# wesselb/stheno

Measured on NVIDIA H100. Metric: log-marginal-likelihoods/sec (n=16384 fp64 EQ), higher is better.
Workload: dtype f64

## Files before the change

stheno_b200/csrc/common.cuh:

```cuda
#pragma once
#include <cuda_runtime.h>
#include <stdint.h>

#include <atomic>
#include <mutex>

#include "../../include/gpk.h"

namespace gpk {

extern long long g_launch_count;

inline int cuda_rc(cudaError_t e) { return e == cudaSuccess ? 0 : -1000 - (int)e; }

#define GPK_CHECK_LAUNCH()                                                  \
  do {                                                                      \
    if (const int rc__ = ::gpk::cuda_rc(cudaGetLastError())) return rc__; \
  } while (0)

#define GPK_COUNT_LAUNCH() (++::gpk::g_launch_count)

template <auto Kernel>
int opt_in_smem(int bytes) {
  static std::atomic<int> set[64];
  static std::mutex mu;
  int dev = 0;
  if (const int rc = cuda_rc(cudaGetDevice(&dev))) return rc;
  if (dev >= 64) return GPK_ERR_UNSUPPORTED;
  if (bytes <= set[dev].load(std::memory_order_acquire)) return 0;
  std::lock_guard<std::mutex> lock(mu);
  if (bytes <= set[dev].load(std::memory_order_relaxed)) return 0;
  if (const int rc = cuda_rc(cudaFuncSetAttribute(Kernel, cudaFuncAttributeMaxDynamicSharedMemorySize, bytes))) return rc;
  set[dev].store(bytes, std::memory_order_release);
  return 0;
}

template <typename T>
__device__ __forceinline__ T t_exp(T v) {
  return sizeof(T) == 8 ? (T)exp((double)v) : (T)expf((float)v);
}
template <typename T>
__device__ __forceinline__ T t_sqrt(T v) {
  return sizeof(T) == 8 ? (T)sqrt((double)v) : (T)sqrtf((float)v);
}
template <typename T>
__device__ __forceinline__ T t_rsqrt(T v) {
  return sizeof(T) == 8 ? (T)rsqrt((double)v) : (T)rsqrtf((float)v);
}
template <typename T>
__device__ __forceinline__ T t_log(T v) {
  return sizeof(T) == 8 ? (T)log((double)v) : (T)logf((float)v);
}

__device__ __forceinline__ uint32_t smem_u32(const void* p) {
  return static_cast<uint32_t>(__cvta_generic_to_shared(p));
}

__device__ __forceinline__ void cp_async16(void* smem_dst, const void* gmem_src) {
  asm volatile("cp.async.cg.shared.global [%0], [%1], 16;\n" ::"r"(smem_u32(smem_dst)), "l"(gmem_src));
}
__device__ __forceinline__ void cp_async_commit() { asm volatile("cp.async.commit_group;\n" ::); }
template <int N>
__device__ __forceinline__ void cp_async_wait() {
  asm volatile("cp.async.wait_group %0;\n" ::"n"(N));
}

__device__ __forceinline__ void mbar_init(uint64_t* bar, uint32_t count) {
  asm volatile("mbarrier.init.shared::cta.b64 [%0], %1;\n" ::"r"(smem_u32(bar)), "r"(count));
}
__device__ __forceinline__ void fence_mbar_init() { asm volatile("fence.mbarrier_init.release.cluster;\n" ::); }
__device__ __forceinline__ void fence_proxy_async() { asm volatile("fence.proxy.async.shared::cta;\n" ::); }
__device__ __forceinline__ void mbar_arrive_expect_tx(uint64_t* bar, uint32_t bytes) {
  asm volatile("mbarrier.arrive.expect_tx.shared::cta.b64 _, [%0], %1;\n" ::"r"(smem_u32(bar)), "r"(bytes));
}
__device__ __forceinline__ void mbar_wait(uint64_t* bar, uint32_t phase) {
  asm volatile(
      "{\n"
      ".reg .pred P1;\n"
      "WAIT_LOOP:\n"
      "mbarrier.try_wait.parity.shared::cta.b64 P1, [%0], %1;\n"
      "@P1 bra WAIT_DONE;\n"
      "bra WAIT_LOOP;\n"
      "WAIT_DONE:\n"
      "}\n" ::"r"(smem_u32(bar)),
      "r"(phase)
      : "memory");
}
__device__ __forceinline__ uint32_t cluster_ctarank() {
  uint32_t r;
  asm volatile("mov.u32 %0, %%cluster_ctarank;\n" : "=r"(r));
  return r;
}
__device__ __forceinline__ void cluster_sync() {
  asm volatile("barrier.cluster.arrive.release;\nbarrier.cluster.wait.acquire;\n" ::: "memory");
}
__device__ __forceinline__ void mbar_arrive_cluster(uint64_t* bar, uint32_t rank) {
  asm volatile(
      "{\n"
      ".reg .b32 remote;\n"
      "mapa.shared::cluster.u32 remote, %0, %1;\n"
      "mbarrier.arrive.shared::cluster.b64 _, [remote];\n"
      "}\n" ::"r"(smem_u32(bar)),
      "r"(rank)
      : "memory");
}
__device__ __forceinline__ void tma_load_3d_multicast(void* dst, const void* map, int c0, int c1, int c2, uint64_t* bar,
                                                      uint16_t cta_mask) {
  asm volatile(
      "cp.async.bulk.tensor.3d.shared::cluster.global.mbarrier::complete_tx::bytes.multicast::cluster [%0], [%1, {%2, %3, "
      "%4}], [%5], %6;\n" ::"r"(smem_u32(dst)),
      "l"(map), "r"(c0), "r"(c1), "r"(c2), "r"(smem_u32(bar)), "h"(cta_mask)
      : "memory");
}
__device__ __forceinline__ void bulk_copy_g2s(void* smem_dst, const void* gmem_src, uint32_t bytes, uint64_t* bar) {
  asm volatile(
      "cp.async.bulk.shared::cluster.global.mbarrier::complete_tx::bytes [%0], [%1], %2, [%3];\n" ::"r"(
          smem_u32(smem_dst)),
      "l"(gmem_src), "r"(bytes), "r"(smem_u32(bar))
      : "memory");
}

__device__ __forceinline__ void dmma884(double& c0, double& c1, double a, double b) {
  asm("mma.sync.aligned.m8n8k4.row.col.f64.f64.f64.f64 {%0,%1}, {%2}, {%3}, {%0,%1};\n"
               : "+d"(c0), "+d"(c1)
               : "d"(a), "d"(b));
}

template <typename T>
__device__ __forceinline__ T warp_sum(T v) {
#pragma unroll
  for (int o = 16; o > 0; o >>= 1) v += __shfl_xor_sync(0xffffffffu, v, o);
  return v;
}


int kernel_rows(const gpk_kernel_desc* desc, const double* xg, int64_t xg_gstride, int64_t n, const double* yg,
                int64_t yg_gstride, int64_t n2, int32_t d, double* out, int64_t ldo, cudaStream_t stream);
int kernel_rows(const gpk_kernel_desc* desc, const float* xg, int64_t xg_gstride, int64_t n, const float* yg,
                int64_t yg_gstride, int64_t n2, int32_t d, float* out, int64_t ldo, cudaStream_t stream);

int row_dot_sq(const double* V, int64_t ldv, int64_t rows, int64_t n_cols, const double* b, double* dot, double* sq,
               cudaStream_t stream);
int row_dot_sq(const float* V, int64_t ldv, int64_t rows, int64_t n_cols, const float* b, float* dot, float* sq,
               cudaStream_t stream);

int gemm_nt(int64_t M, int64_t N, int64_t K, double alpha, const double* A, int64_t lda, int64_t a_bs, const double* B,
            int64_t ldb, int64_t b_bs, double beta, double* C, int64_t ldc, int64_t c_bs, int32_t lower, int32_t batch,
            int32_t S, void* ws, int64_t ws_bytes, cudaStream_t stream);
int gemm_nt(int64_t M, int64_t N, int64_t K, float alpha, const float* A, int64_t lda, int64_t a_bs, const float* B,
            int64_t ldb, int64_t b_bs, float beta, float* C, int64_t ldc, int64_t c_bs, int32_t lower, int32_t batch,
            int32_t S, void* ws, int64_t ws_bytes, cudaStream_t stream);
bool prof_enabled();
void prof_begin(cudaStream_t stream, double flops, int kind);
void prof_end(cudaStream_t stream);

int trsm_right(const double* L, int64_t ldl, int64_t n_pad, double* B, int64_t ldb, int64_t rows, int32_t S, void* ws,
               int64_t ws_bytes, cudaStream_t stream);
int trsm_right(const float* L, int64_t ldl, int64_t n_pad, float* B, int64_t ldb, int64_t rows, int32_t S, void* ws,
               int64_t ws_bytes, cudaStream_t stream);

int oz_check_emulation(int32_t S, const void* ws);
int64_t oz_ws_bytes(int64_t rows, int64_t K, int32_t S);
int oz_slice_panel(const double* P, int64_t ldp, int64_t rows, int64_t K, void* ws, int64_t cap_rows, int32_t S,
                   cudaStream_t stream);
int oz_gemm_sliced(int64_t M, int64_t N, int64_t K, double alpha, const void* wsA, int64_t capA, int64_t rowA,
                   const void* wsB, int64_t capB, int64_t rowB, double beta, double* C, int64_t ldc, int32_t lower,
                   int32_t S, cudaStream_t stream);
int gemm_nt_f64_emulated(int64_t M, int64_t N, int64_t K, double alpha, const double* A, int64_t lda, const double* B,
                         int64_t ldb, double beta, double* C, int64_t ldc, int32_t lower, int32_t S, void* ws,
                         int64_t ws_bytes, cudaStream_t stream);

int gemm_nt_f32_tc(int64_t M, int64_t N, int64_t K, float alpha, const float* A, int64_t lda, int64_t a_bs, const float* B,
                   int64_t ldb, int64_t b_bs, float beta, float* C, int64_t ldc, int64_t c_bs, int32_t lower,
                   int32_t batch, cudaStream_t stream);
int syrk_f64_tf32x3(int64_t M, int64_t N, int64_t K, const float* ws_rows, double* C, int64_t ldc, cudaStream_t stream);
int convert_panel_f32(const double* P, int64_t ldp, int64_t rows, int64_t K, float* ws, cudaStream_t stream);

}
```

stheno_b200/csrc/gemm.cu:

```cuda
#include <vector>

#include "common.cuh"

namespace gpk {

constexpr int GM_BM = 128, GM_BN = 128, GM_BK = 16, GM_THREADS = 256;

template <typename T>
struct GemmParams {
  int64_t M, N, K;
  T alpha, beta;
  const T* A;
  int64_t lda, a_bs;
  const T* B;
  int64_t ldb, b_bs;
  T* C;
  int64_t ldc, c_bs;
  int32_t lower;
  int32_t tiles_m, tiles_n;
};

__device__ __forceinline__ void tile_coords(int id, int tiles_m, int tiles_n, int& tm, int& tn) {
  const int GROUP = 8;
  const int per_group = GROUP * tiles_n;
  const int group = id / per_group;
  const int first_m = group * GROUP;
  const int gsize = min(tiles_m - first_m, GROUP);
  const int r = id - group * per_group;
  tm = first_m + r % gsize;
  tn = r / gsize;
}

constexpr int G2_THREADS = 512;

struct Gemm2Params {
  int64_t K;
  double alpha, beta;
  const double* A;
  int64_t lda, a_bs;
  const double* B;
  int64_t ldb, b_bs;
  double* C;
  int64_t ldc, c_bs;
  int32_t lower, tiles_m, tiles_n, n_groups;
  int32_t tiles_per_batch, total_tiles;
};

__host__ __device__ __forceinline__ int g2_lower_tiles(int rows, int tiles_n) {
  const int tri = rows < tiles_n ? rows : tiles_n;
  return tri * (tri + 1) / 2 + (rows - tri) * tiles_n;
}

__device__ __forceinline__ void g2_decode(const Gemm2Params& p, int idx, int& b, int& tm, int& tn) {
  b = idx / p.tiles_per_batch;
  int r = idx - b * p.tiles_per_batch;
  if (!p.lower) {
    tile_coords(r, p.tiles_m, p.tiles_n, tm, tn);
    return;
  }
  int g = 0;
  while (g + 1 < p.n_groups && g2_lower_tiles(8 * (g + 1), p.tiles_n) <= r) ++g;
  r -= g2_lower_tiles(8 * g, p.tiles_n);
  const int first = g * 8;
  const int gsize = min(p.tiles_m - first, 8);
  const int c0 = min(first, p.tiles_n);
  if (r < c0 * gsize) {
    tn = r / gsize;
    tm = first + r - tn * gsize;
    return;
  }
  r -= c0 * gsize;
  for (int c = 0; c < gsize; ++c) {
    const int cnt = gsize - c;
    if (r < cnt) {
      tn = first + c;
      tm = tn + r;
      return;
    }
    r -= cnt;
  }
  tn = 0;
  tm = first;
}

template <int BK, int STAGES>
__global__ void __launch_bounds__(G2_THREADS, 1) gemm_nt_f64_v2_kernel(const __grid_constant__ Gemm2Params p) {
  constexpr int K8 = BK / 8;
  constexpr int STAGE_ELEMS = GM_BM * BK;
  constexpr int RB = K8 * 64;
  constexpr int GPR = BK / 2;
  constexpr int ROWS_PER_PASS = G2_THREADS / GPR;
  constexpr int PASSES = GM_BM / ROWS_PER_PASS;
  const int tid = threadIdx.x, lane = tid & 31, warp = tid >> 5;
  const int wm = warp >> 2, wn = warp & 3;
  extern __shared__ __align__(16) double gm_smem[];
  double* As = gm_smem;
  double* Bs = gm_smem + STAGES * STAGE_ELEMS;

  const int KT = (int)(p.K / BK);
  const int my_tiles = (p.total_tiles - (int)blockIdx.x + (int)gridDim.x - 1) / (int)gridDim.x;
  const int total_iters = my_tiles * KT;

  const int ld_row = tid / GPR, ld_g = tid % GPR;
  const int ld_off = (ld_row >> 3) * RB + ((ld_g >> 2) * 32 + (ld_row & 7) * 4 + (ld_g & 3)) * 2;
  int ld_it = 0, ld_kt = 0, ld_tile = blockIdx.x, ld_slot = 0;
  const double *ld_a = nullptr, *ld_b = nullptr;
  auto load_next = [&]() {
    if (ld_it < total_iters) {
      if (ld_kt == 0) {
        int b, tm, tn;
        g2_decode(p, ld_tile, b, tm, tn);
        ld_a = p.A + (int64_t)b * p.a_bs + ((int64_t)tm * GM_BM + ld_row) * p.lda + ld_g * 2;
        ld_b = p.B + (int64_t)b * p.b_bs + ((int64_t)tn * GM_BN + ld_row) * p.ldb + ld_g * 2;
      }
      double* as = As + ld_slot * STAGE_ELEMS + ld_off;
      double* bs = Bs + ld_slot * STAGE_ELEMS + ld_off;
      const int64_t koff = (int64_t)ld_kt * BK;
#pragma unroll
      for (int i = 0; i < PASSES; ++i) {
        cp_async16(as + i * (ROWS_PER_PASS / 8) * RB, ld_a + (int64_t)i * ROWS_PER_PASS * p.lda + koff);
        cp_async16(bs + i * (ROWS_PER_PASS / 8) * RB, ld_b + (int64_t)i * ROWS_PER_PASS * p.ldb + koff);
      }
      ++ld_it;
      if (++ld_slot == STAGES) ld_slot = 0;
      if (++ld_kt == KT) {
        ld_kt = 0;
        ld_tile += gridDim.x;
      }
    }
    cp_async_commit();
  };

#pragma unroll
  for (int s = 0; s < STAGES - 1; ++s) load_next();

  double acc[4][4][2];
  int slot = 0;
  const int frag_a = (wm * 4) * RB + lane * 2, frag_b = (wn * 4) * RB + lane * 2;
  for (int t = 0; t < my_tiles; ++t) {
    int b, tm, tn;
    g2_decode(p, (int)blockIdx.x + t * (int)gridDim.x, b, tm, tn);
#pragma unroll
    for (int i = 0; i < 4; ++i)
#pragma unroll
      for (int j = 0; j < 4; ++j) acc[i][j][0] = acc[i][j][1] = 0.0;

    for (int kt = 0; kt < KT; ++kt) {
      cp_async_wait<STAGES - 2>();
      __syncthreads();
      const double* as = As + slot * STAGE_ELEMS + frag_a;
      const double* bs = Bs + slot * STAGE_ELEMS + frag_b;
#pragma unroll
      for (int k8 = 0; k8 < K8; ++k8) {
        double2 a[4], bb[4];
#pragma unroll
        for (int i = 0; i < 4; ++i) a[i] = *reinterpret_cast<const double2*>(as + i * RB + k8 * 64);
#pragma unroll
        for (int j = 0; j < 4; ++j) bb[j] = *reinterpret_cast<const double2*>(bs + j * RB + k8 * 64);
#pragma unroll
        for (int i = 0; i < 4; ++i)
#pragma unroll
          for (int j = 0; j < 4; ++j) dmma884(acc[i][j][0], acc[i][j][1], a[i].x, bb[j].x);
        if (k8 == 0) load_next();
#pragma unroll
        for (int i = 0; i < 4; ++i)
#pragma unroll
          for (int j = 0; j < 4; ++j) dmma884(acc[i][j][0], acc[i][j][1], a[i].y, bb[j].y);
      }
      if (++slot == STAGES) slot = 0;
    }

    double* Cg = p.C + (int64_t)b * p.c_bs + ((int64_t)tm * GM_BM + wm * 32 + (lane >> 2)) * p.ldc +
                 (int64_t)tn * GM_BN + wn * 32 + 2 * (lane & 3);
    const double alpha = p.alpha, beta = p.beta;
    if (beta != 0.0) {
      double2 old[4][4];
#pragma unroll
      for (int i = 0; i < 4; ++i)
#pragma unroll
        for (int j = 0; j < 4; ++j) old[i][j] = *reinterpret_cast<const double2*>(Cg + (int64_t)i * 8 * p.ldc + j * 8);
#pragma unroll
      for (int i = 0; i < 4; ++i)
#pragma unroll
        for (int j = 0; j < 4; ++j) {
          double2 v;
          v.x = fma(alpha, acc[i][j][0], beta * old[i][j].x);
          v.y = fma(alpha, acc[i][j][1], beta * old[i][j].y);
          *reinterpret_cast<double2*>(Cg + (int64_t)i * 8 * p.ldc + j * 8) = v;
        }
    } else {
#pragma unroll
      for (int i = 0; i < 4; ++i)
#pragma unroll
        for (int j = 0; j < 4; ++j)
          *reinterpret_cast<double2*>(Cg + (int64_t)i * 8 * p.ldc + j * 8) =
              make_double2(alpha * acc[i][j][0], alpha * acc[i][j][1]);
    }
  }
  cp_async_wait<0>();
}

constexpr int G3_BN = 64, G3_THREADS = 256;

template <int BK, int STAGES>
__global__ void __launch_bounds__(G3_THREADS, 2) gemm_nt_f64_v3_kernel(const GemmParams<double> p) {
  constexpr int K8 = BK / 8;
  constexpr int RB = K8 * 64;
  constexpr int A_ELEMS = GM_BM * BK, B_ELEMS = G3_BN * BK;
  constexpr int GPR = BK / 2;
  constexpr int ROWS_PER_PASS = G3_THREADS / GPR;
  constexpr int A_PASSES = GM_BM / ROWS_PER_PASS, B_PASSES = G3_BN / ROWS_PER_PASS;
  int tm, tn;
  tile_coords(blockIdx.x, p.tiles_m, p.tiles_n, tm, tn);
  if (p.lower && tn * G3_BN >= (tm + 1) * GM_BM) return;
  const int b = blockIdx.y;
  const int tid = threadIdx.x, lane = tid & 31, warp = tid >> 5;
  const int wm = warp >> 1, wn = warp & 1;
  extern __shared__ __align__(16) double gm_smem[];
  double* As = gm_smem;
  double* Bs = gm_smem + STAGES * A_ELEMS;

  const int ld_row = tid / GPR, ld_g = tid % GPR;
  const int ld_off = (ld_row >> 3) * RB + ((ld_g >> 2) * 32 + (ld_row & 7) * 4 + (ld_g & 3)) * 2;
  const double* ld_a = p.A + (int64_t)b * p.a_bs + ((int64_t)tm * GM_BM + ld_row) * p.lda + ld_g * 2;
  const double* ld_b = p.B + (int64_t)b * p.b_bs + ((int64_t)tn * G3_BN + ld_row) * p.ldb + ld_g * 2;
  const int KT = (int)(p.K / BK);
  int ld_kt = 0, ld_slot = 0;
  auto load_next = [&]() {
    if (ld_kt < KT) {
      double* as = As + ld_slot * A_ELEMS + ld_off;
      double* bs = Bs + ld_slot * B_ELEMS + ld_off;
      const int64_t koff = (int64_t)ld_kt * BK;
#pragma unroll
      for (int i = 0; i < A_PASSES; ++i)
        cp_async16(as + i * (ROWS_PER_PASS / 8) * RB, ld_a + (int64_t)i * ROWS_PER_PASS * p.lda + koff);
#pragma unroll
      for (int i = 0; i < B_PASSES; ++i)
        cp_async16(bs + i * (ROWS_PER_PASS / 8) * RB, ld_b + (int64_t)i * ROWS_PER_PASS * p.ldb + koff);
      ++ld_kt;
      if (++ld_slot == STAGES) ld_slot = 0;
    }
    cp_async_commit();
  };
#pragma unroll
  for (int s = 0; s < STAGES - 1; ++s) load_next();

  double acc[4][4][2];
#pragma unroll
  for (int i = 0; i < 4; ++i)
#pragma unroll
    for (int j = 0; j < 4; ++j) acc[i][j][0] = acc[i][j][1] = 0.0;

  int slot = 0;
  const int frag_a = (wm * 4) * RB + lane * 2, frag_b = (wn * 4) * RB + lane * 2;
  for (int kt = 0; kt < KT; ++kt) {
    cp_async_wait<STAGES - 2>();
    __syncthreads();
    const double* as = As + slot * A_ELEMS + frag_a;
    const double* bs = Bs + slot * B_ELEMS + frag_b;
#pragma unroll
    for (int k8 = 0; k8 < K8; ++k8) {
      double2 a[4], bb[4];
#pragma unroll
      for (int i = 0; i < 4; ++i) a[i] = *reinterpret_cast<const double2*>(as + i * RB + k8 * 64);
#pragma unroll
      for (int j = 0; j < 4; ++j) bb[j] = *reinterpret_cast<const double2*>(bs + j * RB + k8 * 64);
#pragma unroll
      for (int i = 0; i < 4; ++i)
#pragma unroll
        for (int j = 0; j < 4; ++j) dmma884(acc[i][j][0], acc[i][j][1], a[i].x, bb[j].x);
      if (k8 == 0) load_next();
#pragma unroll
      for (int i = 0; i < 4; ++i)
#pragma unroll
        for (int j = 0; j < 4; ++j) dmma884(acc[i][j][0], acc[i][j][1], a[i].y, bb[j].y);
    }
    if (++slot == STAGES) slot = 0;
  }
  cp_async_wait<0>();

  double* Cg = p.C + (int64_t)b * p.c_bs + ((int64_t)tm * GM_BM + wm * 32 + (lane >> 2)) * p.ldc +
               (int64_t)tn * G3_BN + wn * 32 + 2 * (lane & 3);
  const double alpha = p.alpha, beta = p.beta;
  if (beta != 0.0) {
    double2 old[4][4];
#pragma unroll
    for (int i = 0; i < 4; ++i)
#pragma unroll
      for (int j = 0; j < 4; ++j) old[i][j] = *reinterpret_cast<const double2*>(Cg + (int64_t)i * 8 * p.ldc + j * 8);
#pragma unroll
    for (int i = 0; i < 4; ++i)
#pragma unroll
      for (int j = 0; j < 4; ++j) {
        double2 v;
        v.x = fma(alpha, acc[i][j][0], beta * old[i][j].x);
        v.y = fma(alpha, acc[i][j][1], beta * old[i][j].y);
        *reinterpret_cast<double2*>(Cg + (int64_t)i * 8 * p.ldc + j * 8) = v;
      }
  } else {
#pragma unroll
    for (int i = 0; i < 4; ++i)
#pragma unroll
      for (int j = 0; j < 4; ++j)
        *reinterpret_cast<double2*>(Cg + (int64_t)i * 8 * p.ldc + j * 8) =
            make_double2(alpha * acc[i][j][0], alpha * acc[i][j][1]);
  }
}

constexpr int SG_BK = 16;

__global__ void __launch_bounds__(GM_THREADS, 2) gemm_nt_f32_kernel(const GemmParams<float> p) {
  int tm, tn;
  tile_coords(blockIdx.x, p.tiles_m, p.tiles_n, tm, tn);
  if (p.lower && tn > tm) return;
  const int b = blockIdx.y;
  const int tid = threadIdx.x;
  __shared__ __align__(16) float As[2][SG_BK][GM_BM + 4];
  __shared__ __align__(16) float Bs[2][SG_BK][GM_BN + 4];

  const float* Ag = p.A + (int64_t)b * p.a_bs + (int64_t)tm * GM_BM * p.lda;
  const float* Bg = p.B + (int64_t)b * p.b_bs + (int64_t)tn * GM_BN * p.ldb;

  const int lr = tid >> 2, lk = (tid & 3) * 4;
  float4 ra[2], rb[2];
  auto gload = [&](int kt) {
#pragma unroll
    for (int i = 0; i < 2; ++i) {
      ra[i] = *reinterpret_cast<const float4*>(Ag + (int64_t)(lr + 64 * i) * p.lda + (int64_t)kt * SG_BK + lk);
      rb[i] = *reinterpret_cast<const float4*>(Bg + (int64_t)(lr + 64 * i) * p.ldb + (int64_t)kt * SG_BK + lk);
    }
  };
  auto sstore = [&](int buf) {
#pragma unroll
    for (int i = 0; i < 2; ++i) {
      const int r = lr + 64 * i;
      As[buf][lk + 0][r] = ra[i].x;
      As[buf][lk + 1][r] = ra[i].y;
      As[buf][lk + 2][r] = ra[i].z;
      As[buf][lk + 3][r] = ra[i].w;
      Bs[buf][lk + 0][r] = rb[i].x;
      Bs[buf][lk + 1][r] = rb[i].y;
      Bs[buf][lk + 2][r] = rb[i].z;
      Bs[buf][lk + 3][r] = rb[i].w;
    }
  };

  const int tx = tid & 15, ty = tid >> 4;
  float acc[8][8];
#pragma unroll
  for (int i = 0; i < 8; ++i)
#pragma unroll
    for (int j = 0; j < 8; ++j) acc[i][j] = 0.f;

  const int KT = (int)(p.K / SG_BK);
  gload(0);
  sstore(0);
  __syncthreads();
  for (int kt = 0; kt < KT; ++kt) {
    const int buf = kt & 1;
    if (kt + 1 < KT) gload(kt + 1);
#pragma unroll
    for (int k = 0; k < SG_BK; ++k) {
      const float4 a0 = *reinterpret_cast<const float4*>(&As[buf][k][ty * 4]);
      const float4 a1 = *reinterpret_cast<const float4*>(&As[buf][k][64 + ty * 4]);
      const float4 b0 = *reinterpret_cast<const float4*>(&Bs[buf][k][tx * 4]);
      const float4 b1 = *reinterpret_cast<const float4*>(&Bs[buf][k][64 + tx * 4]);
      const float av[8] = {a0.x, a0.y, a0.z, a0.w, a1.x, a1.y, a1.z, a1.w};
      const float bv[8] = {b0.x, b0.y, b0.z, b0.w, b1.x, b1.y, b1.z, b1.w};
#pragma unroll
      for (int i = 0; i < 8; ++i)
#pragma unroll
        for (int j = 0; j < 8; ++j) acc[i][j] = fmaf(av[i], bv[j], acc[i][j]);
    }
    if (kt + 1 < KT) {
      sstore(buf ^ 1);
      __syncthreads();
    }
  }

  float* Cg = p.C + (int64_t)b * p.c_bs + (int64_t)tm * GM_BM * p.ldc + (int64_t)tn * GM_BN;
  const float alpha = p.alpha, beta = p.beta;
#pragma unroll
  for (int i = 0; i < 8; ++i) {
    const int r = (i < 4) ? ty * 4 + i : 64 + ty * 4 + (i - 4);
#pragma unroll
    for (int jh = 0; jh < 2; ++jh) {
      float4* cp = reinterpret_cast<float4*>(Cg + (int64_t)r * p.ldc + jh * 64 + tx * 4);
      float4 v;
      if (beta != 0.f) {
        const float4 o = *cp;
        v.x = fmaf(alpha, acc[i][jh * 4 + 0], beta * o.x);
        v.y = fmaf(alpha, acc[i][jh * 4 + 1], beta * o.y);
        v.z = fmaf(alpha, acc[i][jh * 4 + 2], beta * o.z);
        v.w = fmaf(alpha, acc[i][jh * 4 + 3], beta * o.w);
      } else {
        v.x = alpha * acc[i][jh * 4 + 0];
        v.y = alpha * acc[i][jh * 4 + 1];
        v.z = alpha * acc[i][jh * 4 + 2];
        v.w = alpha * acc[i][jh * 4 + 3];
      }
      *cp = v;
    }
  }
}

template <typename T>
static int check_gemm_args(int64_t M, int64_t N, int64_t K, const T* A, int64_t lda, const T* B, int64_t ldb, T* C,
                           int64_t ldc, int32_t batch) {
  if (M < 0 || N < 0 || K < 0 || batch < 1 || !A || !B || !C) return GPK_ERR_ARG;
  if (M % GM_BM || N % GM_BN || K % GM_BK) return GPK_ERR_ARG;
  if (lda < K || ldb < K || ldc < N) return GPK_ERR_ARG;
  const int64_t al = 16 / sizeof(T);
  if (lda % al || ldb % al || ldc % al) return GPK_ERR_ALIGN;
  if ((reinterpret_cast<uintptr_t>(A) | reinterpret_cast<uintptr_t>(B) | reinterpret_cast<uintptr_t>(C)) % 16)
    return GPK_ERR_ALIGN;
  return 0;
}

struct GemmProfile {
  bool enabled = false;
  std::vector<cudaEvent_t> ev;
  std::vector<double> flops;
  std::vector<int> kind;
};
static GemmProfile g_prof;

bool prof_enabled() { return g_prof.enabled; }
void prof_begin(cudaStream_t s, double flops, int kind) {
// ... 131 lines not shown
```

stheno_b200/csrc/potrf.cu:

```cuda
#include <stdlib.h>

#include "common.cuh"

namespace gpk {

constexpr int NB = 128;

template <typename T>
__global__ void __launch_bounds__(256, 1)
potrf_leaf_kernel(T* __restrict__ A, int64_t lda, int64_t a_bs, T* __restrict__ logdet, int32_t* __restrict__ info,
                  int32_t pivot_base) {
  const int bidx = blockIdx.x;
  A += (int64_t)bidx * a_bs;
  const int tid = threadIdx.x, ti = tid >> 4, tk = tid & 15;
  __shared__ T colbuf[2][NB];
  __shared__ T diag[NB];
  __shared__ T red[8];

  T acc[8][8];
#pragma unroll
  for (int a = 0; a < 8; ++a)
#pragma unroll
    for (int b = 0; b < 8; ++b) acc[a][b] = A[(int64_t)(ti + 16 * a) * lda + tk + 16 * b];

// ... 165 lines not shown
    } else if (b > 0) {
      const int pb = b - 1;
      const int nblk = (4 - b) * (3 - b) / 2;
      if (nblk > 0) {
        const int U = (RL_WARPS - 1) / nblk;
        const int u = warp - 1;
        if (u < U * nblk) {
          const int blk = u / U, q = u - blk * U;
          int r, c;
          if (b == 1) {
            c = (blk == 2) ? 3 : 2;
            r = (blk == 0) ? 2 : 3;
          } else {
            r = c = 3;
          }
          rl_update_cols(S, r, c, pb, (q * 32) / U, ((q + 1) * 32) / U, lane);
        }
      }
    }
    __syncthreads();
    if (dbg) dbg[dbg_i++] = clock64();
    if (b == 3) break;
    const int nrows = NB - 32 * (b + 1);
    if (tid < nrows) {
      double* rowp = S + (32 * (b + 1) + tid) * RL_LD + 32 * b;
      double x[32];
#pragma unroll
      for (int k = 0; k < 32; k += 2) {
        const double2 v = *reinterpret_cast<const double2*>(rowp + k);
        x[k] = v.x;
        x[k + 1] = v.y;
      }
#pragma unroll
      for (int j = 0; j < 32; ++j) {
        x[j] *= dinv[j];
#pragma unroll
        for (int k = j + 1; k < 32; ++k) x[k] = fma(-x[j], colT[j * 32 + k], x[k]);
      }
#pragma unroll
      for (int k = 0; k < 32; k += 2) *reinterpret_cast<double2*>(rowp + k) = make_double2(x[k], x[k + 1]);
    }
    __syncthreads();
    if (dbg) dbg[dbg_i++] = clock64();
    {
      const int c = b + 1, nblk = 4 - c, U = RL_WARPS / nblk;
      if (warp < U * nblk) {
        const int blk = warp / U, q = warp - blk * U;
        rl_update_cols(S, c + blk, c, b, (q * 32) / U, ((q + 1) * 32) / U, lane);
      }
    }
    __syncthreads();
    if (dbg) dbg[dbg_i++] = clock64();
  }

  for (int gi = tid; gi < NB * NB / 2; gi += RL_THREADS) {
    const int row = gi >> 6, k = (gi & 63) * 2;
    if (k <= row) {
      const double2 v = *reinterpret_cast<const double2*>(S + row * RL_LD + k);
      T* dst = A + (int64_t)row * lda + k;
      if (k + 1 <= row) {
        if (sizeof(T) == 8) *reinterpret_cast<double2*>(dst) = v;
        else *reinterpret_cast<float2*>(dst) = make_float2((float)v.x, (float)v.y);
      } else {
        dst[0] = (T)v.x;
      }
    }
  }
  if (logdet != nullptr && warp == 0) {
    const double s = warp_sum(logsum);
    if (lane == 0) atomicAdd(logdet + bidx, (T)(2.0 * s));
  }
  if (dbg) dbg[dbg_i++] = clock64();
}

constexpr int TL_LD = NB + 2;

template <typename T>
__global__ void __launch_bounds__(256, 1)
trsm_leaf_kernel(const T* __restrict__ L, int64_t ldl, int64_t l_bs, T* __restrict__ B, int64_t ldb, int64_t b_bs) {
  extern __shared__ __align__(16) unsigned char tl_smem[];
  T* Lt = reinterpret_cast<T*>(tl_smem);
  T* invd = Lt + NB * TL_LD;
  T* xbuf = invd + NB;
  const int tid = threadIdx.x;
  const int bidx = blockIdx.y;
  L += (int64_t)bidx * l_bs;
  B += (int64_t)bidx * b_bs + (int64_t)blockIdx.x * 64 * ldb;

  for (int idx = tid; idx < NB * NB; idx += 256) {
    const int k = idx >> 7, j = idx & 127;
    const T v = (j <= k) ? L[(int64_t)k * ldl + j] : T(0);
    Lt[k * TL_LD + j] = v;
    if (j == k) invd[j] = T(1) / v;
  }
  const int r = tid & 63, cg = tid >> 6;
  T a[32];
  {
    const T* src = B + (int64_t)r * ldb + 32 * cg;
#pragma unroll
    for (int q = 0; q < 32; ++q) a[q] = src[q];
  }
  __syncthreads();

  int buf = 0;
  for (int step = 0; step < NB; ++step) {
    const int j = NB - 1 - step;
    const int cgj = j >> 5, jj = j & 31;
    if (cg == cgj) {
      T x = T(0);
#pragma unroll
      for (int q = 0; q < 32; ++q) x = (q == jj) ? a[q] : x;
      x *= invd[j];
#pragma unroll
      for (int q = 0; q < 32; ++q) a[q] = (q == jj) ? x : a[q];
      xbuf[buf * 64 + r] = x;
    }
    __syncthreads();
    if (cg <= cgj) {
      const T x = xbuf[buf * 64 + r];
      const T* lrow = Lt + j * TL_LD + 32 * cg;
#pragma unroll
      for (int q = 0; q < 32; ++q) {
        const bool ok = (cg != cgj) || (q < jj);
        if (ok) a[q] -= x * lrow[q];
      }
    }
    buf ^= 1;
  }
  {
    T* dst = B + (int64_t)r * ldb + 32 * cg;
#pragma unroll
    for (int q = 0; q < 32; ++q) dst[q] = a[q];
  }
}

constexpr int TC_ROWS = 128;
constexpr int TC_THREADS = 512;
constexpr int TC_SMEM = (NB * NB + 8 * 16 * 17) * (int)sizeof(double);

__device__ __forceinline__ int frag_index(int n, int k) {
  return (((n >> 3) * 16 + (k >> 3)) * 32 + (n & 7) * 4 + ((k & 7) >> 1)) * 2 + (k & 1);
}

template <typename T>
__global__ void __launch_bounds__(TC_THREADS, 1)
trsm_leaf_tc_kernel(const T* __restrict__ L, int64_t ldl, int64_t l_bs, T* __restrict__ B, int64_t ldb, int64_t b_bs,
                    int32_t rows_per_cta) {
  extern __shared__ __align__(16) unsigned char tc_smem[];
  double* Ls = reinterpret_cast<double*>(tc_smem);
  double* Ld = Ls + NB * NB;
  const int tid = threadIdx.x, lane = tid & 31, warp = tid >> 5;
  L += (int64_t)blockIdx.y * l_bs;
  B += (int64_t)blockIdx.y * b_bs + (int64_t)blockIdx.x * rows_per_cta * ldb;

#pragma unroll
  for (int gi = tid; gi < NB * NB / 2; gi += TC_THREADS) {
    const int c = gi >> 6, g = gi & 63;
    const int k = 2 * g;
    double2 v = make_double2(0.0, 0.0);
    if (k <= c) {
      const T* src = L + (int64_t)c * ldl + k;
      if (sizeof(T) == 8) {
        v = *reinterpret_cast<const double2*>(src);
      } else {
        const float2 f = *reinterpret_cast<const float2*>(src);
        v = make_double2((double)f.x, (double)f.y);
      }
      if (k + 1 > c) v.y = 0.0;
    }
    *reinterpret_cast<double2*>(Ls + frag_index(c, k)) = v;
    if ((c >> 4) == (k >> 4)) {
      double* d = Ld + ((c >> 4) * 16 + (c & 15)) * 17 + (k & 15);
      d[0] = v.x;
      d[1] = v.y;
    }
  }
  __syncthreads();
  if (warp < 8) {
    double* Lb = Ld + warp * 16 * 17;
    if (lane < 16) Lb[lane * 17 + 16] = 1.0 / Lb[lane * 17 + lane];
    __syncwarp();
    if (lane < 16) {
      double x[16];
#pragma unroll
      for (int i = 0; i < 16; ++i) {
        double s = (i == lane) ? 1.0 : 0.0;
#pragma unroll
        for (int k = 0; k < 16; ++k)
          if (k < i) s -= Lb[i * 17 + k] * x[k];
        x[i] = (i >= lane) ? s * Lb[i * 17 + 16] : 0.0;
      }
#pragma unroll
      for (int i = 0; i < 16; ++i) Ls[frag_index(warp * 16 + i, warp * 16 + lane)] = x[i];
    }
  }
  __syncthreads();

  if (warp * 8 >= rows_per_cta) return;
  double acc[16][2];
  T* Bw = B + (int64_t)(warp * 8 + (lane >> 2)) * ldb + 2 * (lane & 3);
#pragma unroll
  for (int cb = 0; cb < 16; ++cb) {
    acc[cb][0] = (double)Bw[cb * 8];
    acc[cb][1] = (double)Bw[cb * 8 + 1];
  }
  const double* Lf = Ls + lane * 2;
#pragma unroll
  for (int jb = 0; jb < 8; ++jb) {
    double x[2][2] = {{0.0, 0.0}, {0.0, 0.0}};
#pragma unroll
    for (int nb = 0; nb < 2; ++nb)
#pragma unroll
      for (int kg = 0; kg < 2; ++kg) {
        if (kg > nb) continue;
        const double2 b = *reinterpret_cast<const double2*>(Lf + ((2 * jb + nb) * 16 + 2 * jb + kg) * 64);
        dmma884(x[nb][0], x[nb][1], acc[2 * jb + kg][0], b.x);
        dmma884(x[nb][0], x[nb][1], acc[2 * jb + kg][1], b.y);
      }
    acc[2 * jb][0] = x[0][0];
    acc[2 * jb][1] = x[0][1];
    acc[2 * jb + 1][0] = x[1][0];
    acc[2 * jb + 1][1] = x[1][1];
    const double nx[2][2] = {{-x[0][0], -x[0][1]}, {-x[1][0], -x[1][1]}};
#pragma unroll
    for (int kg = 0; kg < 2; ++kg) {
      double2 b[16];
#pragma unroll
      for (int cb = 2 * jb + 2; cb < 16; ++cb)
        b[cb] = *reinterpret_cast<const double2*>(Lf + (cb * 16 + 2 * jb + kg) * 64);
#pragma unroll
      for (int cb = 2 * jb + 2; cb < 16; ++cb) dmma884(acc[cb][0], acc[cb][1], nx[kg][0], b[cb].x);
#pragma unroll
      for (int cb = 2 * jb + 2; cb < 16; ++cb) dmma884(acc[cb][0], acc[cb][1], nx[kg][1], b[cb].y);
    }
  }
#pragma unroll
  for (int cb = 0; cb < 16; ++cb) {
    Bw[cb * 8] = (T)acc[cb][0];
    Bw[cb * 8 + 1] = (T)acc[cb][1];
  }
}

template <typename T>
static int trsm_leaf_fwd(const T* L, int64_t ldl, int64_t l_bs, T* B, int64_t ldb, int64_t b_bs, int64_t rows,
                         int32_t batch, cudaStream_t stream) {
  if (rows % TC_ROWS) return GPK_ERR_ARG;
  if (rows == 0) return 0;
  if (const int rc = opt_in_smem<trsm_leaf_tc_kernel<T>>(TC_SMEM)) return rc;
  dim3 grid((unsigned)(rows / TC_ROWS), (unsigned)batch);
  trsm_leaf_tc_kernel<T><<<grid, TC_THREADS, TC_SMEM, stream>>>(L, ldl, l_bs, B, ldb, b_bs, TC_ROWS);
  GPK_COUNT_LAUNCH();
  GPK_CHECK_LAUNCH();
  return 0;
}

template <typename T>
__global__ void __launch_bounds__(256)
diag_syrk_kernel(const T* __restrict__ X, int64_t ldx, int64_t x_bs, T* __restrict__ D, int64_t ldd, int64_t d_bs) {
  const int lane = threadIdx.x & 31;
  const int g = blockIdx.x * 8 + (threadIdx.x >> 5);
  int rb = (int)((sqrtf(8.f * (float)g + 1.f) - 1.f) * 0.5f);
  while (rb * (rb + 1) / 2 > g) --rb;
  while ((rb + 1) * (rb + 2) / 2 <= g) ++rb;
  const int cb = g - rb * (rb + 1) / 2;
  X += (int64_t)blockIdx.y * x_bs;
  D += (int64_t)blockIdx.y * d_bs;
  const T* Xa = X + (int64_t)(rb * 8 + (lane >> 2)) * ldx + 2 * (lane & 3);
  const T* Xb = X + (int64_t)(cb * 8 + (lane >> 2)) * ldx + 2 * (lane & 3);
  double a[16][2], b[16][2];
#pragma unroll
  for (int kg = 0; kg < 16; ++kg) {
    a[kg][0] = (double)Xa[kg * 8];
    a[kg][1] = (double)Xa[kg * 8 + 1];
    b[kg][0] = (double)Xb[kg * 8];
    b[kg][1] = (double)Xb[kg * 8 + 1];
  }
  T* Dp = D + (int64_t)(rb * 8 + (lane >> 2)) * ldd + cb * 8 + 2 * (lane & 3);
  const double c0 = (double)Dp[0], c1 = (double)Dp[1];
  double d0[2] = {0.0, 0.0}, d1[2] = {0.0, 0.0};
#pragma unroll
  for (int kg = 0; kg < 8; ++kg) {
    dmma884(d0[0], d0[1], a[kg][0], b[kg][0]);
    dmma884(d1[0], d1[1], a[kg + 8][0], b[kg + 8][0]);
    dmma884(d0[0], d0[1], a[kg][1], b[kg][1]);
    dmma884(d1[0], d1[1], a[kg + 8][1], b[kg + 8][1]);
  }
  Dp[0] = (T)(c0 - (d0[0] + d1[0]));
  Dp[1] = (T)(c1 - (d0[1] + d1[1]));
}

template <typename T>
static int launch_diag_step(const T* L, int64_t ldl, int64_t l_bs, T* B, int64_t ldb, int64_t b_bs, T* D, int64_t ldd,
                            int64_t d_bs, int32_t batch, cudaStream_t stream) {
  if (const int rc = opt_in_smem<trsm_leaf_tc_kernel<T>>(TC_SMEM)) return rc;
  trsm_leaf_tc_kernel<T><<<dim3(4, (unsigned)batch), TC_THREADS, TC_SMEM, stream>>>(L, ldl, l_bs, B, ldb, b_bs, 32);
  GPK_COUNT_LAUNCH();
  GPK_CHECK_LAUNCH();
  diag_syrk_kernel<T><<<dim3(17, (unsigned)batch), 256, 0, stream>>>(B, ldb, b_bs, D, ldd, d_bs);
  GPK_COUNT_LAUNCH();
  GPK_CHECK_LAUNCH();
  return 0;
}

template <typename T>
static int launch_potrf_leaf(T* A, int64_t lda, int64_t a_bs, T* logdet, int32_t* info, int32_t pivot_base,
                             int32_t batch, cudaStream_t stream) {
// ... 421 lines not shown
```

stheno_b200/csrc/util.cu:

```cuda
#include <math.h>

#include "common.cuh"

namespace gpk {

long long g_launch_count = 0;

template <typename T>
__global__ void logpdf_finish_kernel(const T* __restrict__ a, int64_t lda, int64_t a_bs, int64_t n, int64_t n_cols,
                                     int32_t k, const T* __restrict__ logdet, T* __restrict__ out) {
  const int c = blockIdx.x, b = blockIdx.y;
  const T* row = a + (int64_t)b * a_bs + (int64_t)c * lda;
  T s = T(0);
  for (int64_t j = threadIdx.x; j < n_cols; j += blockDim.x) {
    const T v = row[j];
    s = fma(v, v, s);
  }
  __shared__ T red[32];
  s = warp_sum(s);
  if ((threadIdx.x & 31) == 0) red[threadIdx.x >> 5] = s;
  __syncthreads();
  if (threadIdx.x == 0) {
    T t = T(0);
    for (int w = 0; w < (int)(blockDim.x >> 5); ++w) t += red[w];
    const T log2pi = T(1.8378770664093454835606594728112);
    out[(int64_t)b * k + c] = -(logdet[b] + (T)n * log2pi + t) / T(2);
  }
}

template <typename T>
__global__ void row_dot_sq_kernel(const T* __restrict__ V, int64_t ldv, int64_t v_bs, int64_t rows, int64_t n_cols,
                                  const T* __restrict__ bvec, int64_t b_bs, T* __restrict__ dot, T* __restrict__ sq,
                                  int64_t o_bs) {
  const int bidx = blockIdx.y;
  const int64_t r = (int64_t)blockIdx.x * (blockDim.x >> 5) + (threadIdx.x >> 5);
  if (r >= rows) return;
  const int lane = threadIdx.x & 31;
  const T* row = V + (int64_t)bidx * v_bs + r * ldv;
  const T* bv = bvec ? bvec + (int64_t)bidx * b_bs : nullptr;
  T sd = T(0), ss = T(0);
  for (int64_t j = lane; j < n_cols; j += 32) {
    const T v = row[j];
    ss = fma(v, v, ss);
    if (bv) sd = fma(v, bv[j], sd);
  }
  sd = warp_sum(sd);
  ss = warp_sum(ss);
  if (lane == 0) {
    if (dot) dot[(int64_t)bidx * o_bs + r] = sd;
    if (sq) sq[(int64_t)bidx * o_bs + r] = ss;
  }
}

template <typename T>
__global__ void pad_copy_kernel(const T* __restrict__ src, int64_t lds, int64_t s_bs, int64_t rows, int64_t cols,
                                T* __restrict__ dst, int64_t ldd, int64_t d_bs, int64_t rows_pad, int64_t cols_pad,
                                T diag_add, int32_t pad_identity) {
  const int64_t c = (int64_t)blockIdx.x * blockDim.x + threadIdx.x;
  const int b = blockIdx.z;
  if (c >= cols_pad) return;
  for (int64_t r = blockIdx.y; r < rows_pad; r += gridDim.y) {
    T v;
    if (r < rows && c < cols) {
      v = src[(int64_t)b * s_bs + r * lds + c];
      if (r == c) v += diag_add;
    } else {
      v = (pad_identity && r == c) ? T(1) : T(0);
    }
    dst[(int64_t)b * d_bs + r * ldd + c] = v;
  }
}

template <typename T>
__global__ void symmetrize_kernel(T* __restrict__ A, int64_t lda, int64_t a_bs, int64_t n) {
  __shared__ T tile[32][33];
  const int tr = blockIdx.y, tc = blockIdx.x;
  if (tc > tr) return;
  A += (int64_t)blockIdx.z * a_bs;
  const int tx = threadIdx.x, ty = threadIdx.y;
  for (int i = ty; i < 32; i += 8) {
    const int64_t r = (int64_t)tr * 32 + i, c = (int64_t)tc * 32 + tx;
    tile[i][tx] = (r < n && c < n) ? A[r * lda + c] : T(0);
  }
  __syncthreads();
  for (int i = ty; i < 32; i += 8) {
    const int64_t r = (int64_t)tc * 32 + i, c = (int64_t)tr * 32 + tx;
    if (r < n && c < n && c > r) A[r * lda + c] = tile[tx][i];
  }
}

template <typename T>
__global__ void transpose_kernel(const T* __restrict__ src, int64_t lds, int64_t s_bs, int64_t rows, int64_t cols,
                                 T* __restrict__ dst, int64_t ldd, int64_t d_bs) {
  __shared__ T tile[32][33];
  src += (int64_t)blockIdx.z * s_bs;
  dst += (int64_t)blockIdx.z * d_bs;
  const int tx = threadIdx.x, ty = threadIdx.y;
  const int64_t r0 = (int64_t)blockIdx.x * 32;
  for (int64_t c0 = (int64_t)blockIdx.y * 32; c0 < cols; c0 += (int64_t)gridDim.y * 32) {
    for (int i = ty; i < 32; i += 8) {
      const int64_t r = r0 + i, c = c0 + tx;
      tile[i][tx] = (r < rows && c < cols) ? src[r * lds + c] : T(0);
    }
    __syncthreads();
    for (int i = ty; i < 32; i += 8) {
      const int64_t r = c0 + i, c = r0 + tx;
      if (r < cols && c < rows) dst[r * ldd + c] = tile[tx][i];
    }
    __syncthreads();
  }
}

__global__ void dmma_probe_kernel(double* out, int iters, double a, double b) {
  double c[8][2];
#pragma unroll
  for (int i = 0; i < 8; ++i) {
    c[i][0] = threadIdx.x;
    c[i][1] = i;
  }
  for (int it = 0; it < iters; ++it) {
#pragma unroll
    for (int i = 0; i < 8; ++i) dmma884(c[i][0], c[i][1], a, b);
  }
  double s = 0;
#pragma unroll
  for (int i = 0; i < 8; ++i) s += c[i][0] + c[i][1];
  out[blockIdx.x * blockDim.x + threadIdx.x] = s;
}

int row_dot_sq(const double* V, int64_t ldv, int64_t rows, int64_t n_cols, const double* b, double* dot, double* sq,
               cudaStream_t stream) {
  return gpk_row_dot_sq_f64(V, ldv, 0, rows, n_cols, b, 0, dot, sq, 0, 1, stream);
}
int row_dot_sq(const float* V, int64_t ldv, int64_t rows, int64_t n_cols, const float* b, float* dot, float* sq,
               cudaStream_t stream) {
  return gpk_row_dot_sq_f32(V, ldv, 0, rows, n_cols, b, 0, dot, sq, 0, 1, stream);
}

}

#define GPK_DEFINE_UTILS(SUF, T)                                                                                       \
  int gpk_logpdf_finish_##SUF(const T* a, int64_t lda, int64_t a_bstride, int64_t n, int64_t n_cols, int32_t k,        \
                              const T* logdet, T* out, int32_t batch, void* stream) {                                  \
    if (!a || !logdet || !out || k < 1 || batch < 1 || n_cols < 0) return GPK_ERR_ARG;                                 \
    dim3 grid((unsigned)k, (unsigned)batch);                                                                           \
    gpk::logpdf_finish_kernel<T><<<grid, 512, 0, (cudaStream_t)stream>>>(a, lda, a_bstride, n, n_cols, k, logdet, out); \
    GPK_COUNT_LAUNCH();                                                                                                \
    GPK_CHECK_LAUNCH();                                                                                                \
    return 0;                                                                                                          \
  }                                                                                                                    \
  int gpk_row_dot_sq_##SUF(const T* V, int64_t ldv, int64_t v_bstride, int64_t rows, int64_t n_cols, const T* b,       \
                           int64_t b_bstride, T* dot, T* sq, int64_t o_bstride, int32_t batch, void* stream) {         \
    if (!V || rows < 0 || n_cols < 0 || batch < 1) return GPK_ERR_ARG;                                                 \
    if (rows == 0) return 0;                                                                                           \
    dim3 grid((unsigned)((rows + 7) / 8), (unsigned)batch);                                                            \
    gpk::row_dot_sq_kernel<T><<<grid, 256, 0, (cudaStream_t)stream>>>(V, ldv, v_bstride, rows, n_cols, b, b_bstride,   \
                                                                     dot, sq, o_bstride);                              \
    GPK_COUNT_LAUNCH();                                                                                                \
    GPK_CHECK_LAUNCH();                                                                                                \
    return 0;                                                                                                          \
  }                                                                                                                    \
  int gpk_pad_copy_##SUF(const T* src, int64_t lds, int64_t s_bstride, int64_t rows, int64_t cols, T* dst,             \
                         int64_t ldd, int64_t d_bstride, int64_t rows_pad, int64_t cols_pad, double diag_add,          \
                         int32_t pad_identity, int32_t batch, void* stream) {                                          \
    if (!dst || rows < 0 || cols < 0 || rows_pad < rows || cols_pad < cols || batch < 1) return GPK_ERR_ARG;           \
    if (rows_pad == 0 || cols_pad == 0) return 0;                                                                      \
    dim3 grid((unsigned)((cols_pad + 255) / 256), (unsigned)(rows_pad < 65535 ? rows_pad : 65535), (unsigned)batch);   \
    gpk::pad_copy_kernel<T><<<grid, 256, 0, (cudaStream_t)stream>>>(src, lds, s_bstride, rows, cols, dst, ldd,         \
                                                                   d_bstride, rows_pad, cols_pad, (T)diag_add,         \
                                                                   pad_identity);                                      \
    GPK_COUNT_LAUNCH();                                                                                                \
    GPK_CHECK_LAUNCH();                                                                                                \
    return 0;                                                                                                          \
  }                                                                                                                    \
  int gpk_symmetrize_##SUF(T* A, int64_t lda, int64_t a_bstride, int64_t n, int32_t batch, void* stream) {             \
    if (!A || n < 0 || batch < 1) return GPK_ERR_ARG;                                                                  \
    if (n == 0) return 0;                                                                                              \
    const unsigned t = (unsigned)((n + 31) / 32);                                                                      \
    dim3 grid(t, t, (unsigned)batch), block(32, 8);                                                                    \
    gpk::symmetrize_kernel<T><<<grid, block, 0, (cudaStream_t)stream>>>(A, lda, a_bstride, n);                         \
    GPK_COUNT_LAUNCH();                                                                                                \
    GPK_CHECK_LAUNCH();                                                                                                \
    return 0;                                                                                                          \
  }                                                                                                                    \
  int gpk_transpose_##SUF(const T* src, int64_t lds, int64_t s_bstride, int64_t rows, int64_t cols, T* dst,            \
                          int64_t ldd, int64_t d_bstride, int32_t batch, void* stream) {                               \
    if (!src || !dst || rows < 0 || cols < 0 || batch < 1) return GPK_ERR_ARG;                                         \
    if (rows == 0 || cols == 0) return 0;                                                                              \
    const int64_t col_tiles = (cols + 31) / 32;                                                                        \
    dim3 grid((unsigned)((rows + 31) / 32), (unsigned)(col_tiles < 65535 ? col_tiles : 65535), (unsigned)batch),       \
        block(32, 8);                                                                                                  \
    gpk::transpose_kernel<T><<<grid, block, 0, (cudaStream_t)stream>>>(src, lds, s_bstride, rows, cols, dst, ldd,      \
                                                                      d_bstride);                                      \
    GPK_COUNT_LAUNCH();                                                                                                \
    GPK_CHECK_LAUNCH();                                                                                                \
    return 0;                                                                                                          \
  }

extern "C" {

GPK_DEFINE_UTILS(f64, double)
GPK_DEFINE_UTILS(f32, float)

int gpk_version(void) { return GPK_VERSION; }
int64_t gpk_round_up(int64_t n) { return (n + GPK_TILE - 1) / GPK_TILE * GPK_TILE; }
int64_t gpk_launch_count(void) { return gpk::g_launch_count; }
void gpk_launch_count_reset(void) { gpk::g_launch_count = 0; }

double gpk_probe_dmma_tflops(void) {
  int dev = 0, sms = 0;
  if (cudaGetDevice(&dev) != cudaSuccess) return -1.0;
  if (cudaDeviceGetAttribute(&sms, cudaDevAttrMultiProcessorCount, dev) != cudaSuccess) return -1.0;
  double* out = nullptr;
  const int threads = 256, iters = 20000;
  if (cudaMalloc(&out, sizeof(double) * sms * threads) != cudaSuccess) return -2.0;
  cudaEvent_t e0, e1;
  cudaEventCreate(&e0);
  cudaEventCreate(&e1);
  gpk::dmma_probe_kernel<<<sms, threads>>>(out, iters, 1.0000001, 0.9999999);
  cudaDeviceSynchronize();
  float best = 1e30f;
  for (int rep = 0; rep < 3; ++rep) {
    cudaEventRecord(e0);
    gpk::dmma_probe_kernel<<<sms, threads>>>(out, iters, 1.0000001, 0.9999999);
    cudaEventRecord(e1);
    cudaEventSynchronize(e1);
    float ms = 0.f;
    cudaEventElapsedTime(&ms, e0, e1);
    if (ms < best) best = ms;
  }
  cudaEventDestroy(e0);
  cudaEventDestroy(e1);
  cudaFree(out);
  if (cudaGetLastError() != cudaSuccess) return -3.0;
  return 512.0 * 8 * iters * (threads / 32) * sms / (best * 1e-3) / 1e12;
}
}
```

Baseline: 25.40.

## Switch FP64 GEMM inner loop to m16n8k16 DMMA with fragment-ordered A tiles

```diff
diff --git a/stheno_b200/csrc/common.cuh b/stheno_b200/csrc/common.cuh
--- a/stheno_b200/csrc/common.cuh
+++ b/stheno_b200/csrc/common.cuh
@@ -58,6 +58,10 @@
 
 __device__ __forceinline__ void cp_async16(void* smem_dst, const void* gmem_src) {
   asm volatile("cp.async.cg.shared.global [%0], [%1], 16;\n" ::"r"(smem_u32(smem_dst)), "l"(gmem_src));
+}
+__device__ __forceinline__ void prefetch_l2(const void* p) { asm volatile("prefetch.global.L2 [%0];\n" ::"l"(p)); }
+__device__ __forceinline__ void cp_async8(void* smem_dst, const void* gmem_src) {
+  asm volatile("cp.async.ca.shared.global [%0], [%1], 8;\n" ::"r"(smem_u32(smem_dst)), "l"(gmem_src));
 }
 __device__ __forceinline__ void cp_async_commit() { asm volatile("cp.async.commit_group;\n" ::); }
 template <int N>
@@ -126,6 +130,21 @@
                : "d"(a), "d"(b));
 }
 
+__device__ __forceinline__ void dmma16816(double& c0, double& c1, double& c2, double& c3, double a0, double a1, double a2,
+                                          double a3, double a4, double a5, double a6, double a7, double b0, double b1,
+                                          double b2, double b3) {
+  asm("mma.sync.aligned.m16n8k16.row.col.f64.f64.f64.f64 {%0,%1,%2,%3}, {%4,%5,%6,%7,%8,%9,%10,%11}, {%12,%13,%14,%15}, "
+      "{%0,%1,%2,%3};\n"
+      : "+d"(c0), "+d"(c1), "+d"(c2), "+d"(c3)
+      : "d"(a0), "d"(a1), "d"(a2), "d"(a3), "d"(a4), "d"(a5), "d"(a6), "d"(a7), "d"(b0), "d"(b1), "d"(b2), "d"(b3));
+}
+
+__device__ __forceinline__ void dmma16816_frag(double (&c0)[2], double (&c1)[2], const double2 (&a)[4],
+                                               const double2 (&b)[2]) {
+  dmma16816(c0[0], c0[1], c1[0], c1[1], a[0].x, a[0].y, a[1].x, a[1].y, a[2].x, a[2].y, a[3].x, a[3].y, b[0].x, b[0].y,
+            b[1].x, b[1].y);
+}
+
 template <typename T>
 __device__ __forceinline__ T warp_sum(T v) {
 #pragma unroll
diff --git a/stheno_b200/csrc/gemm.cu b/stheno_b200/csrc/gemm.cu
--- a/stheno_b200/csrc/gemm.cu
+++ b/stheno_b200/csrc/gemm.cu
@@ -83,6 +83,26 @@
   tm = first;
 }
 
+struct ALoad {
+  int row, smem;
+};
+template <int BK>
+__device__ __forceinline__ ALoad a_load_slot(int tid) {
+  const int t = tid & 3, rid = tid >> 2, half = rid & 1, g = (rid >> 1) & 7, rb = rid >> 4;
+  return {16 * rb + 8 * half + g, rb * 16 * BK + 2 * (g * 4 + t) + half};
+}
+template <int BK, int THREADS>
+__device__ __forceinline__ void a_load_stage(double* dst, const double* src, int64_t lda) {
+#pragma unroll
+  for (int r = 0; r < GM_BM / (THREADS / 4); ++r)
+#pragma unroll
+    for (int s = 0; s < BK / 16; ++s)
+#pragma unroll
+      for (int q = 0; q < 4; ++q)
+        cp_async8(dst + r * (THREADS / 64) * 16 * BK + (s * 4 + q) * 64,
+                  src + (int64_t)r * (THREADS / 4) * lda + 16 * s + 8 * (q >> 1) + (q & 1));
+}
+
 template <int BK, int STAGES>
 __global__ void __launch_bounds__(G2_THREADS, 1) gemm_nt_f64_v2_kernel(const __grid_constant__ Gemm2Params p) {
   constexpr int K8 = BK / 8;
@@ -103,6 +123,7 @@
 
   const int ld_row = tid / GPR, ld_g = tid % GPR;
   const int ld_off = (ld_row >> 3) * RB + ((ld_g >> 2) * 32 + (ld_row & 7) * 4 + (ld_g & 3)) * 2;
+  const ALoad a_ld = a_load_slot<BK>(tid);
   int ld_it = 0, ld_kt = 0, ld_tile = blockIdx.x, ld_slot = 0;
   const double *ld_a = nullptr, *ld_b = nullptr;
   auto load_next = [&]() {
@@ -110,17 +131,15 @@
       if (ld_kt == 0) {
         int b, tm, tn;
         g2_decode(p, ld_tile, b, tm, tn);
-        ld_a = p.A + (int64_t)b * p.a_bs + ((int64_t)tm * GM_BM + ld_row) * p.lda + ld_g * 2;
+        ld_a = p.A + (int64_t)b * p.a_bs + ((int64_t)tm * GM_BM + a_ld.row) * p.lda + 2 * (tid & 3);
         ld_b = p.B + (int64_t)b * p.b_bs + ((int64_t)tn * GM_BN + ld_row) * p.ldb + ld_g * 2;
       }
-      double* as = As + ld_slot * STAGE_ELEMS + ld_off;
       double* bs = Bs + ld_slot * STAGE_ELEMS + ld_off;
       const int64_t koff = (int64_t)ld_kt * BK;
-#pragma unroll
-      for (int i = 0; i < PASSES; ++i) {
-        cp_async16(as + i * (ROWS_PER_PASS / 8) * RB, ld_a + (int64_t)i * ROWS_PER_PASS * p.lda + koff);
+      a_load_stage<BK, G2_THREADS>(As + ld_slot * STAGE_ELEMS + a_ld.smem, ld_a + koff, p.lda);
+#pragma unroll
+      for (int i = 0; i < PASSES; ++i)
         cp_async16(bs + i * (ROWS_PER_PASS / 8) * RB, ld_b + (int64_t)i * ROWS_PER_PASS * p.ldb + koff);
-      }
       ++ld_it;
       if (++ld_slot == STAGES) ld_slot = 0;
       if (++ld_kt == KT) {
@@ -136,10 +155,16 @@
 
   double acc[4][4][2];
   int slot = 0;
-  const int frag_a = (wm * 4) * RB + lane * 2, frag_b = (wn * 4) * RB + lane * 2;
+  const int frag_a = (wm * 2) * 16 * BK + lane * 2, frag_b = (wn * 4) * RB + lane * 2;
   for (int t = 0; t < my_tiles; ++t) {
     int b, tm, tn;
     g2_decode(p, (int)blockIdx.x + t * (int)gridDim.x, b, tm, tn);
+    if (p.beta != 0.0) {
+      const double* c = p.C + (int64_t)b * p.c_bs + ((int64_t)tm * GM_BM + (tid >> 2)) * p.ldc + (int64_t)tn * GM_BN +
+                        (tid & 3) * 32;
+      prefetch_l2(c);
+      prefetch_l2(c + 16);
+    }
 #pragma unroll
     for (int i = 0; i < 4; ++i)
 #pragma unroll
@@ -151,21 +176,22 @@
       const double* as = As + slot * STAGE_ELEMS + frag_a;
       const double* bs = Bs + slot * STAGE_ELEMS + frag_b;
 #pragma unroll
-      for (int k8 = 0; k8 < K8; ++k8) {
-        double2 a[4], bb[4];
-#pragma unroll
-        for (int i = 0; i < 4; ++i) a[i] = *reinterpret_cast<const double2*>(as + i * RB + k8 * 64);
-#pragma unroll
-        for (int j = 0; j < 4; ++j) bb[j] = *reinterpret_cast<const double2*>(bs + j * RB + k8 * 64);
-#pragma unroll
-        for (int i = 0; i < 4; ++i)
-#pragma unroll
-          for (int j = 0; j < 4; ++j) dmma884(acc[i][j][0], acc[i][j][1], a[i].x, bb[j].x);
-        if (k8 == 0) load_next();
-#pragma unroll
-        for (int i = 0; i < 4; ++i)
-#pragma unroll
-          for (int j = 0; j < 4; ++j) dmma884(acc[i][j][0], acc[i][j][1], a[i].y, bb[j].y);
+      for (int k16 = 0; k16 < K8 / 2; ++k16) {
+        double2 a[2][4];
+#pragma unroll
+        for (int i = 0; i < 2; ++i)
+#pragma unroll
+          for (int q = 0; q < 4; ++q)
+            a[i][q] = *reinterpret_cast<const double2*>(as + ((i * (BK / 16) + k16) * 4 + q) * 64);
+#pragma unroll
+        for (int j = 0; j < 4; ++j) {
+          double2 bb[2];
+#pragma unroll
+          for (int h = 0; h < 2; ++h) bb[h] = *reinterpret_cast<const double2*>(bs + j * RB + (2 * k16 + h) * 64);
+          dmma16816_frag(acc[0][j], acc[1][j], a[0], bb);
+          dmma16816_frag(acc[2][j], acc[3][j], a[1], bb);
+          if (k16 == 0 && j == 1) load_next();
+        }
       }
       if (++slot == STAGES) slot = 0;
     }
@@ -209,7 +235,7 @@
   constexpr int A_ELEMS = GM_BM * BK, B_ELEMS = G3_BN * BK;
   constexpr int GPR = BK / 2;
   constexpr int ROWS_PER_PASS = G3_THREADS / GPR;
-  constexpr int A_PASSES = GM_BM / ROWS_PER_PASS, B_PASSES = G3_BN / ROWS_PER_PASS;
+  constexpr int B_PASSES = G3_BN / ROWS_PER_PASS;
   int tm, tn;
   tile_coords(blockIdx.x, p.tiles_m, p.tiles_n, tm, tn);
   if (p.lower && tn * G3_BN >= (tm + 1) * GM_BM) return;
@@ -222,18 +248,16 @@
 
   const int ld_row = tid / GPR, ld_g = tid % GPR;
   const int ld_off = (ld_row >> 3) * RB + ((ld_g >> 2) * 32 + (ld_row & 7) * 4 + (ld_g & 3)) * 2;
-  const double* ld_a = p.A + (int64_t)b * p.a_bs + ((int64_t)tm * GM_BM + ld_row) * p.lda + ld_g * 2;
+  const ALoad a_ld = a_load_slot<BK>(tid);
+  const double* ld_a = p.A + (int64_t)b * p.a_bs + ((int64_t)tm * GM_BM + a_ld.row) * p.lda + 2 * (tid & 3);
   const double* ld_b = p.B + (int64_t)b * p.b_bs + ((int64_t)tn * G3_BN + ld_row) * p.ldb + ld_g * 2;
   const int KT = (int)(p.K / BK);
   int ld_kt = 0, ld_slot = 0;
   auto load_next = [&]() {
     if (ld_kt < KT) {
-      double* as = As + ld_slot * A_ELEMS + ld_off;
       double* bs = Bs + ld_slot * B_ELEMS + ld_off;
       const int64_t koff = (int64_t)ld_kt * BK;
-#pragma unroll
-      for (int i = 0; i < A_PASSES; ++i)
-        cp_async16(as + i * (ROWS_PER_PASS / 8) * RB, ld_a + (int64_t)i * ROWS_PER_PASS * p.lda + koff);
+      a_load_stage<BK, G3_THREADS>(As + ld_slot * A_ELEMS + a_ld.smem, ld_a + koff, p.lda);
 #pragma unroll
       for (int i = 0; i < B_PASSES; ++i)
         cp_async16(bs + i * (ROWS_PER_PASS / 8) * RB, ld_b + (int64_t)i * ROWS_PER_PASS * p.ldb + koff);
@@ -252,28 +276,29 @@
     for (int j = 0; j < 4; ++j) acc[i][j][0] = acc[i][j][1] = 0.0;
 
   int slot = 0;
-  const int frag_a = (wm * 4) * RB + lane * 2, frag_b = (wn * 4) * RB + lane * 2;
+  const int frag_a = (wm * 2) * 16 * BK + lane * 2, frag_b = (wn * 4) * RB + lane * 2;
   for (int kt = 0; kt < KT; ++kt) {
     cp_async_wait<STAGES - 2>();
     __syncthreads();
     const double* as = As + slot * A_ELEMS + frag_a;
     const double* bs = Bs + slot * B_ELEMS + frag_b;
 #pragma unroll
-    for (int k8 = 0; k8 < K8; ++k8) {
-      double2 a[4], bb[4];
-#pragma unroll
-      for (int i = 0; i < 4; ++i) a[i] = *reinterpret_cast<const double2*>(as + i * RB + k8 * 64);
-#pragma unroll
-      for (int j = 0; j < 4; ++j) bb[j] = *reinterpret_cast<const double2*>(bs + j * RB + k8 * 64);
-#pragma unroll
-      for (int i = 0; i < 4; ++i)
-#pragma unroll
-        for (int j = 0; j < 4; ++j) dmma884(acc[i][j][0], acc[i][j][1], a[i].x, bb[j].x);
-      if (k8 == 0) load_next();
-#pragma unroll
-      for (int i = 0; i < 4; ++i)
-#pragma unroll
-        for (int j = 0; j < 4; ++j) dmma884(acc[i][j][0], acc[i][j][1], a[i].y, bb[j].y);
+    for (int k16 = 0; k16 < K8 / 2; ++k16) {
+      double2 a[2][4];
+#pragma unroll
+      for (int i = 0; i < 2; ++i)
+#pragma unroll
+        for (int q = 0; q < 4; ++q)
+          a[i][q] = *reinterpret_cast<const double2*>(as + ((i * (BK / 16) + k16) * 4 + q) * 64);
+#pragma unroll
+      for (int j = 0; j < 4; ++j) {
+        double2 bb[2];
+#pragma unroll
+        for (int h = 0; h < 2; ++h) bb[h] = *reinterpret_cast<const double2*>(bs + j * RB + (2 * k16 + h) * 64);
+        dmma16816_frag(acc[0][j], acc[1][j], a[0], bb);
+        dmma16816_frag(acc[2][j], acc[3][j], a[1], bb);
+        if (k16 == 0 && j == 1) load_next();
+      }
     }
     if (++slot == STAGES) slot = 0;
   }
diff --git a/stheno_b200/csrc/potrf.cu b/stheno_b200/csrc/potrf.cu
--- a/stheno_b200/csrc/potrf.cu
+++ b/stheno_b200/csrc/potrf.cu
@@ -341,6 +341,11 @@
   const int tid = threadIdx.x, lane = tid & 31, warp = tid >> 5;
   L += (int64_t)blockIdx.y * l_bs;
   B += (int64_t)blockIdx.y * b_bs + (int64_t)blockIdx.x * rows_per_cta * ldb;
+  if (warp * 8 < rows_per_cta) {
+    const char* r = reinterpret_cast<const char*>(B + (int64_t)(warp * 8 + (lane >> 2)) * ldb) + (lane & 3) * 32 * sizeof(T);
+#pragma unroll
+    for (int o = 0; o < 32 * (int)sizeof(T); o += 128) prefetch_l2(r + o);
+  }
 
 #pragma unroll
   for (int gi = tid; gi < NB * NB / 2; gi += TC_THREADS) {
diff --git a/stheno_b200/csrc/util.cu b/stheno_b200/csrc/util.cu
--- a/stheno_b200/csrc/util.cu
+++ b/stheno_b200/csrc/util.cu
@@ -112,19 +112,18 @@
 }
 
 __global__ void dmma_probe_kernel(double* out, int iters, double a, double b) {
-  double c[8][2];
-#pragma unroll
-  for (int i = 0; i < 8; ++i) {
-    c[i][0] = threadIdx.x;
-    c[i][1] = i;
-  }
+  double c[4][4];
+#pragma unroll
+  for (int i = 0; i < 4; ++i)
+#pragma unroll
+    for (int j = 0; j < 4; ++j) c[i][j] = threadIdx.x + j;
   for (int it = 0; it < iters; ++it) {
 #pragma unroll
-    for (int i = 0; i < 8; ++i) dmma884(c[i][0], c[i][1], a, b);
+    for (int i = 0; i < 4; ++i) dmma16816(c[i][0], c[i][1], c[i][2], c[i][3], a, a, a, a, a, a, a, a, b, b, b, b);
   }
   double s = 0;
 #pragma unroll
-  for (int i = 0; i < 8; ++i) s += c[i][0] + c[i][1];
+  for (int i = 0; i < 4; ++i) s += c[i][0] + c[i][1] + c[i][2] + c[i][3];
   out[blockIdx.x * blockDim.x + threadIdx.x] = s;
 }
 
@@ -212,7 +211,7 @@
   if (cudaGetDevice(&dev) != cudaSuccess) return -1.0;
   if (cudaDeviceGetAttribute(&sms, cudaDevAttrMultiProcessorCount, dev) != cudaSuccess) return -1.0;
   double* out = nullptr;
-  const int threads = 256, iters = 20000;
+  const int threads = 256, iters = 2500;
   if (cudaMalloc(&out, sizeof(double) * sms * threads) != cudaSuccess) return -2.0;
   cudaEvent_t e0, e1;
   cudaEventCreate(&e0);
@@ -233,6 +232,6 @@
   cudaEventDestroy(e1);
   cudaFree(out);
   if (cudaGetLastError() != cudaSuccess) return -3.0;
-  return 512.0 * 8 * iters * (threads / 32) * sms / (best * 1e-3) / 1e12;
-}
-}
+  return 4096.0 * 4 * iters * (threads / 32) * sms / (best * 1e-3) / 1e12;
+}
+}
```

Measured after the change: 25.68, median of 6. 1.1% higher.
